# mbzuai-oryx/Video-LLaVA

Hardware: NVIDIA H100
Metric: videos/sec (100-frame CLIP encode + 7B 32-tok decode) (higher is better)
Workload: dtype bf16

## Files before the change

video-llava_b200/csrc/attention_tc.cu:

```cuda
#include "common.cuh"
#include "kernels.h"

#include <stdlib.h>

namespace vcl {

namespace {

constexpr int VA_WG = 2;
constexpr int VA_THREADS = VA_WG * 128;
constexpr int VA_TILE = 64 * 128;
constexpr int VA_KEY_TILES = 5;
constexpr int VA_OFF_K = 0;
constexpr int VA_OFF_VT = VA_OFF_K + VA_KEY_TILES * VA_TILE;
constexpr int VA_OFF_Q = VA_OFF_VT + VA_KEY_TILES * VA_TILE;
constexpr int VA_OFF_P = VA_OFF_Q + VA_WG * VA_TILE;
constexpr int VA_OFF_BAR = VA_OFF_P + VA_WG * VA_KEY_TILES * VA_TILE;
constexpr int VA_SMEM = VA_OFF_BAR + 64 + 1024;
static_assert(VA_SMEM <= 227 * 1024, "shared memory");

__device__ __forceinline__ uint32_t va_sw128(int row, int chunk) {
  return (uint32_t)row * 128u + (uint32_t)((chunk ^ (row & 7)) << 4);
}

__device__ __forceinline__ void named_bar_sync_wg(int id) { asm volatile("bar.sync %0, 128;" ::"r"(id) : "memory"); }

__global__ void __launch_bounds__(VA_THREADS, 1)
attn_vit_tc_kernel(const __grid_constant__ CUtensorMap tmap, const bf16* __restrict__ qkv, bf16* __restrict__ out,
                   int S, int H, int C) {
  extern __shared__ uint8_t smem_raw[];
  const uint32_t raw_addr = smem_u32(smem_raw);
  const uint32_t pad = ((raw_addr + 1023u) & ~1023u) - raw_addr;
  uint8_t* smem = smem_raw + pad;
  const uint32_t sbase = raw_addr + pad;
  const uint32_t kbar = sbase + VA_OFF_BAR;
  auto qbar = [&](int w) { return sbase + VA_OFF_BAR + 8u * (1 + w); };

  const int frame = blockIdx.x / H, h = blockIdx.x - frame * H;
  const int row0 = frame * S;
  const int wg = threadIdx.x >> 7, t = threadIdx.x & 127, lane = threadIdx.x & 31, wq = t >> 5;
  const int n_qt = (S + 63) / 64;
  const int n_kt = (S + 63) / 64;

  if (threadIdx.x == 0) {
    tma_prefetch_desc(&tmap);
    mbar_init(kbar, 1);
    for (int w = 0; w < VA_WG; ++w) mbar_init(qbar(w), 1);
    mbar_fence_init();
  }
  __syncthreads();
  if (threadIdx.x == 0) {
    mbar_arrive_expect_tx(kbar, n_kt * VA_TILE);
    for (int i = 0; i < n_kt; ++i) tma_load_2d(sbase + VA_OFF_K + i * VA_TILE, &tmap, kbar, C + h * 64, row0 + 64 * i);
    for (int w = 0; w < VA_WG && w < n_qt; ++w) {
      mbar_arrive_expect_tx(qbar(w), VA_TILE);
      tma_load_2d(sbase + VA_OFF_Q + w * VA_TILE, &tmap, qbar(w), h * 64, row0 + 64 * w);
    }
  }
  const bf16* vg = qkv + (long long)row0 * 3 * C + 2 * C + h * 64;
  for (int idx = threadIdx.x; idx < VA_KEY_TILES * 64 * 8; idx += VA_THREADS) {
    const int key = idx % (VA_KEY_TILES * 64), c = idx / (VA_KEY_TILES * 64);
    uint4 v = make_uint4(0u, 0u, 0u, 0u);
    if (key < S) v = *reinterpret_cast<const uint4*>(vg + (long long)key * 3 * C + c * 8);
    const uint32_t w4[4] = {v.x, v.y, v.z, v.w};
    uint8_t* tile = smem + VA_OFF_VT + (key >> 6) * VA_TILE;
    const int kc = (key & 63) >> 3, ke = key & 7;
#pragma unroll
    for (int e = 0; e < 8; ++e) {
      const uint16_t hv = (uint16_t)(e & 1 ? w4[e >> 1] >> 16 : w4[e >> 1] & 0xffffu);
      *reinterpret_cast<uint16_t*>(tile + va_sw128(c * 8 + e, kc) + ke * 2) = hv;
    }
  }
  asm volatile("fence.proxy.async.shared::cta;" ::: "memory");
  __syncthreads();
  mbar_wait(kbar, 0);

  const int r0 = 16 * wq + (lane >> 2), c2 = 2 * (lane & 3);
  const bool tail = S > 256;
  uint8_t* P = smem + VA_OFF_P + wg * VA_KEY_TILES * VA_TILE;
  const uint32_t p_addr = sbase + VA_OFF_P + wg * VA_KEY_TILES * VA_TILE;
  const uint32_t q_addr = sbase + VA_OFF_Q + wg * VA_TILE;
  uint32_t qphase = 0;
  float s[128], s2[16], o[32];
  for (int qt = wg; qt < n_qt; qt += VA_WG) {
    mbar_wait(qbar(wg), qphase);
    qphase ^= 1u;
#pragma unroll
    for (int i = 0; i < 128; ++i) s[i] = 0.f;
#pragma unroll
    for (int i = 0; i < 16; ++i) s2[i] = 0.f;
    wgmma_fence();
#pragma unroll
    for (int k = 0; k < 4; ++k) {
      const uint64_t ad = wgmma_desc_k_sw128(q_addr) + 2u * k;
      wgmma_bf16<256>(s, ad, wgmma_desc_k_sw128(sbase + VA_OFF_K) + 2u * k, k > 0 ? 1u : 0u);
      if (tail) wgmma_bf16<32>(s2, ad, wgmma_desc_k_sw128(sbase + VA_OFF_K + 256 * 128) + 2u * k, k > 0 ? 1u : 0u);
    }
    wgmma_commit();
    wgmma_wait<0>();
    wgmma_fence_regs(s);
    wgmma_fence_regs(s2);
    named_bar_sync_wg(1 + wg);
    if (t == 0 && qt + VA_WG < n_qt) {
      mbar_arrive_expect_tx(qbar(wg), VA_TILE);
      tma_load_2d(q_addr, &tmap, qbar(wg), h * 64, row0 + 64 * (qt + VA_WG));
    }
    auto sc = [&](float x, int key) { return key < S ? bf16r(bf16r(x) * 0.125f) : -INFINITY; };
    float m[2] = {-INFINITY, -INFINITY};
    uint32_t sp[64], sp2[8];
    auto pack_sc = [&](const float* a, int i, int key0) {
      const int hh = i & 1, col = key0 + 8 * (i >> 1) + c2;
      const float x0 = sc(a[2 * i], col), x1 = sc(a[2 * i + 1], col + 1);
      m[hh] = fmaxf(m[hh], fmaxf(x0, x1));
      return pack_bf16x2(x0, x1);
    };
    if (tail) {
#pragma unroll
      for (int i = 0; i < 8; ++i) sp2[i] = pack_sc(s2, i, 256);
    }
#pragma unroll
    for (int i = 0; i < 64; ++i) sp[i] = pack_sc(s, i, 0);
    float l[2] = {0.f, 0.f};
#pragma unroll
    for (int r = 0; r < 2; ++r) {
      m[r] = fmaxf(m[r], __shfl_xor_sync(0xffffffffu, m[r], 1));
      m[r] = fmaxf(m[r], __shfl_xor_sync(0xffffffffu, m[r], 2));
    }
    auto put_p = [&](uint32_t x2, int i, int key0) {
      const int hh = i & 1, row = r0 + 8 * hh, col = key0 + 8 * (i >> 1) + c2;
      const float p0 = exp2f((bf16lo(x2) - m[hh]) * 1.4426950408889634f);
      const float p1 = exp2f((bf16hi(x2) - m[hh]) * 1.4426950408889634f);
      l[hh] += p0 + p1;
      *reinterpret_cast<uint32_t*>(P + (col >> 6) * VA_TILE + va_sw128(row, (col & 63) >> 3) + (col & 7) * 2) =
          pack_bf16x2(p0, p1);
    };
#pragma unroll
    for (int i = 0; i < 64; ++i) put_p(sp[i], i, 0);
    if (tail) {
#pragma unroll
      for (int i = 0; i < 8; ++i) put_p(sp2[i], i, 256);
    }
    asm volatile("fence.proxy.async.shared::cta;" ::: "memory");
    named_bar_sync_wg(1 + wg);
#pragma unroll
    for (int i = 0; i < 32; ++i) o[i] = 0.f;
    wgmma_fence();
#pragma unroll
    for (int kk = 0; kk < 16; ++kk)
      wgmma_bf16<64>(o, wgmma_desc_k_sw128(p_addr + (kk >> 2) * VA_TILE) + 2u * (kk & 3),
                     wgmma_desc_k_sw128(sbase + VA_OFF_VT + (kk >> 2) * VA_TILE) + 2u * (kk & 3), kk > 0 ? 1u : 0u);
    if (tail)
      wgmma_bf16<64>(o, wgmma_desc_k_sw128(p_addr + 4 * VA_TILE), wgmma_desc_k_sw128(sbase + VA_OFF_VT + 4 * VA_TILE), 1u);
    wgmma_commit();
    wgmma_wait<0>();
    wgmma_fence_regs(o);
#pragma unroll
    for (int r = 0; r < 2; ++r) {
      l[r] += __shfl_xor_sync(0xffffffffu, l[r], 1);
      l[r] += __shfl_xor_sync(0xffffffffu, l[r], 2);
    }
#pragma unroll
    for (int hh = 0; hh < 2; ++hh) {
      const int q = qt * 64 + r0 + 8 * hh;
      if (q < S) {
        const float inv = 1.0f / l[hh];
        bf16* dst = out + (long long)(row0 + q) * C + h * 64 + c2;
#pragma unroll
        for (int j = 0; j < 8; ++j)
          *reinterpret_cast<uint32_t*>(dst + 8 * j) = pack_bf16x2(o[4 * j + 2 * hh] * inv, o[4 * j + 2 * hh + 1] * inv);
      }
    }
  }
}

}

int init_attention_tc_kernels() {
  VCL_CUDA_OK(cudaFuncSetAttribute(attn_vit_tc_kernel, cudaFuncAttributeMaxDynamicSharedMemorySize, VA_SMEM));
  return 0;
}

bool attention_vit_tc_supported(int S) {
  const bool off = getenv("VCL_VIT_ATTN_FLASH") != nullptr;
  return !off && S >= 129 && S <= 257;
}

int launch_attention_vit_tc(const bf16* qkv, bf16* out, int n_frames, int S, int H, int C, cudaStream_t stream) {
  VCL_REQUIRE(C == H * 64, "attention_vit_tc: head_dim must be 64");
  VCL_REQUIRE(S >= 129 && S <= 257, "attention_vit_tc: S=%d outside 129..257", S);
  VCL_REQUIRE(((uintptr_t)qkv % 16) == 0 && ((uintptr_t)out % 16) == 0, "attention_vit_tc: pointers must be 16-byte aligned");
  CUtensorMap tm;
  if (make_tmap_2d(&tm, qkv, (long long)n_frames * S, 3LL * C, 3LL * C, 64) != 0) return -2;
  attn_vit_tc_kernel<<<n_frames * H, VA_THREADS, VA_SMEM, stream>>>(tm, qkv, out, S, H, C);
  VCL_CUDA_OK(cudaGetLastError());
  count_launches(1);
  return 0;
}

}
```

video-llava_b200/csrc/common.cuh:

```cuda
#pragma once

#include <cuda.h>
#include <cuda_bf16.h>
#include <cuda_fp16.h>
#include <cuda_runtime.h>
#include <stdint.h>

namespace vcl {

typedef __nv_bfloat16 bf16;

void set_last_error(const char* fmt, ...);

#define VCL_CUDA_OK(expr)                                                                      \
  do {                                                                                         \
    cudaError_t _e = (expr);                                                                   \
    if (_e != cudaSuccess) {                                                                   \
      ::vcl::set_last_error("%s:%d: %s -> %s", __FILE__, __LINE__, #expr, cudaGetErrorString(_e)); \
      return -2;                                                                               \
    }                                                                                          \
  } while (0)

#define VCL_REQUIRE(cond, ...)                 \
  do {                                         \
// ... 26 lines not shown
  for (int o = 16; o > 0; o >>= 1) v += __shfl_xor_sync(0xffffffffu, v, o);
  return v;
}
__device__ __forceinline__ float warp_max(float v) {
#pragma unroll
  for (int o = 16; o > 0; o >>= 1) v = fmaxf(v, __shfl_xor_sync(0xffffffffu, v, o));
  return v;
}

__device__ __forceinline__ uint4 ld_nc_v4(const void* p) {
  uint4 r;
  asm volatile("ld.global.nc.L1::no_allocate.v4.u32 {%0,%1,%2,%3}, [%4];"
               : "=r"(r.x), "=r"(r.y), "=r"(r.z), "=r"(r.w)
               : "l"(p));
  return r;
}

__device__ __forceinline__ uint32_t smem_u32(const void* p) {
  return static_cast<uint32_t>(__cvta_generic_to_shared(p));
}

__device__ __forceinline__ void mbar_init(uint32_t bar, uint32_t count) {
  asm volatile("mbarrier.init.shared::cta.b64 [%0], %1;" ::"r"(bar), "r"(count) : "memory");
}
__device__ __forceinline__ void mbar_fence_init() {
  asm volatile("fence.mbarrier_init.release.cluster;" ::: "memory");
  asm volatile("fence.proxy.async.shared::cta;" ::: "memory");
}
__device__ __forceinline__ void mbar_arrive_expect_tx(uint32_t bar, uint32_t bytes) {
  asm volatile("mbarrier.arrive.expect_tx.shared::cta.b64 _, [%0], %1;" ::"r"(bar), "r"(bytes)
               : "memory");
}
__device__ __forceinline__ void mbar_arrive(uint32_t bar) {
  asm volatile("mbarrier.arrive.shared::cta.b64 _, [%0];" ::"r"(bar) : "memory");
}
__device__ __forceinline__ void mbar_wait(uint32_t bar, uint32_t parity) {
  asm volatile(
      "{\n\t"
      ".reg .pred p;\n\t"
      "VCL_WAIT_%=:\n\t"
      "mbarrier.try_wait.parity.shared::cta.b64 p, [%0], %1;\n\t"
      "@p bra VCL_DONE_%=;\n\t"
      "bra VCL_WAIT_%=;\n\t"
      "VCL_DONE_%=:\n\t"
      "}\n" ::"r"(bar),
      "r"(parity)
      : "memory");
}

__device__ __forceinline__ void tma_prefetch_desc(const void* tmap) {
  asm volatile("prefetch.tensormap [%0];" ::"l"(tmap) : "memory");
}
__device__ __forceinline__ void tma_load_2d(uint32_t dst_smem, const void* tmap, uint32_t bar,
                                            int32_t c0, int32_t c1) {
  asm volatile(
      "cp.async.bulk.tensor.2d.shared::cluster.global.mbarrier::complete_tx::bytes"
      " [%0], [%1, {%3, %4}], [%2];" ::"r"(dst_smem),
      "l"(tmap), "r"(bar), "r"(c0), "r"(c1)
      : "memory");
}

__device__ __forceinline__ void tma_prefetch_2d(const void* tmap, int32_t c0, int32_t c1) {
  asm volatile("cp.async.bulk.prefetch.tensor.2d.L2.global.tile [%0, {%1, %2}];" ::"l"(tmap), "r"(c0), "r"(c1)
               : "memory");
}

__device__ __forceinline__ void tma_load_2d_mc(uint32_t dst_smem, const void* tmap, uint32_t bar,
                                               int32_t c0, int32_t c1, uint16_t cta_mask) {
  asm volatile(
      "cp.async.bulk.tensor.2d.shared::cluster.global.mbarrier::complete_tx::bytes.multicast::cluster"
      " [%0], [%1, {%3, %4}], [%2], %5;" ::"r"(dst_smem),
      "l"(tmap), "r"(bar), "r"(c0), "r"(c1), "h"(cta_mask)
      : "memory");
}

__device__ __forceinline__ uint32_t cluster_ctarank() {
  uint32_t r;
  asm volatile("mov.u32 %0, %%cluster_ctarank;" : "=r"(r));
  return r;
}
__device__ __forceinline__ void cluster_sync_all() {
  asm volatile("barrier.cluster.arrive.release.aligned;" ::: "memory");
  asm volatile("barrier.cluster.wait.acquire.aligned;" ::: "memory");
}

__device__ __forceinline__ uint32_t mapa_cluster(uint32_t smem_addr, uint32_t cta_rank) {
  uint32_t r;
  asm volatile("mapa.shared::cluster.u32 %0, %1, %2;" : "=r"(r) : "r"(smem_addr), "r"(cta_rank));
  return r;
}
__device__ __forceinline__ void mbar_arrive_cluster(uint32_t bar_cluster_addr) {
  asm volatile("mbarrier.arrive.release.cluster.shared::cluster.b64 _, [%0];" ::"r"(bar_cluster_addr) : "memory");
}

__device__ __forceinline__ void wgmma_fence() { asm volatile("wgmma.fence.sync.aligned;" ::: "memory"); }
__device__ __forceinline__ void wgmma_commit() { asm volatile("wgmma.commit_group.sync.aligned;" ::: "memory"); }
template <int N>
__device__ __forceinline__ void wgmma_wait() {
  asm volatile("wgmma.wait_group.sync.aligned %0;" ::"n"(N) : "memory");
}
template <int R>
__device__ __forceinline__ void wgmma_fence_regs(float (&d)[R]) {
#pragma unroll
  for (int i = 0; i < R; ++i) asm volatile("" : "+f"(d[i])::"memory");
}
template <int R>
__device__ __forceinline__ void setmaxnreg_inc() { asm volatile("setmaxnreg.inc.sync.aligned.u32 %0;" ::"n"(R)); }
template <int R>
__device__ __forceinline__ void setmaxnreg_dec() { asm volatile("setmaxnreg.dec.sync.aligned.u32 %0;" ::"n"(R)); }

__device__ __forceinline__ uint64_t wgmma_desc_k_sw128(uint32_t smem_addr) {
  uint64_t d = 0;
  d |= (uint64_t)((smem_addr & 0x3ffffu) >> 4);
  d |= (uint64_t)1 << 16;
  d |= (uint64_t)(1024u >> 4) << 32;
  d |= (uint64_t)1 << 62;
  return d;
}

template <int N>
__device__ __forceinline__ void wgmma_bf16(float (&d)[N / 2], uint64_t adesc, uint64_t bdesc, uint32_t accumulate);
template <>
__device__ __forceinline__ void wgmma_bf16<256>(float (&d)[128], uint64_t adesc, uint64_t bdesc, uint32_t accumulate) {
  asm volatile(
      "{\n\t.reg .pred p;\n\tsetp.ne.b32 p, %130, 0;\n\t"
      "wgmma.mma_async.sync.aligned.m64n256k16.f32.bf16.bf16 {%0, %1, %2, %3, %4, %5, %6, %7, %8, %9, %10, %11, %12, %13, %14, %15, %16, %17, %18, %19, %20, %21, %22, %23, %24, %25, %26, %27, %28, %29, %30, %31, %32, %33, %34, %35, %36, %37, %38, %39, %40, %41, %42, %43, %44, %45, %46, %47, %48, %49, %50, %51, %52, %53, %54, %55, %56, %57, %58, %59, %60, %61, %62, %63, %64, %65, %66, %67, %68, %69, %70, %71, %72, %73, %74, %75, %76, %77, %78, %79, %80, %81, %82, %83, %84, %85, %86, %87, %88, %89, %90, %91, %92, %93, %94, %95, %96, %97, %98, %99, %100, %101, %102, %103, %104, %105, %106, %107, %108, %109, %110, %111, %112, %113, %114, %115, %116, %117, %118, %119, %120, %121, %122, %123, %124, %125, %126, %127}, %128, %129, p, 1, 1, 0, 0;\n\t}"
      : "+f"(d[0]), "+f"(d[1]), "+f"(d[2]), "+f"(d[3]), "+f"(d[4]), "+f"(d[5]), "+f"(d[6]), "+f"(d[7]), "+f"(d[8]), "+f"(d[9]), "+f"(d[10]), "+f"(d[11]), "+f"(d[12]), "+f"(d[13]), "+f"(d[14]), "+f"(d[15]), "+f"(d[16]), "+f"(d[17]), "+f"(d[18]), "+f"(d[19]), "+f"(d[20]), "+f"(d[21]), "+f"(d[22]), "+f"(d[23]), "+f"(d[24]), "+f"(d[25]), "+f"(d[26]), "+f"(d[27]), "+f"(d[28]), "+f"(d[29]), "+f"(d[30]), "+f"(d[31]), "+f"(d[32]), "+f"(d[33]), "+f"(d[34]), "+f"(d[35]), "+f"(d[36]), "+f"(d[37]), "+f"(d[38]), "+f"(d[39]), "+f"(d[40]), "+f"(d[41]), "+f"(d[42]), "+f"(d[43]), "+f"(d[44]), "+f"(d[45]), "+f"(d[46]), "+f"(d[47]), "+f"(d[48]), "+f"(d[49]), "+f"(d[50]), "+f"(d[51]), "+f"(d[52]), "+f"(d[53]), "+f"(d[54]), "+f"(d[55]), "+f"(d[56]), "+f"(d[57]), "+f"(d[58]), "+f"(d[59]), "+f"(d[60]), "+f"(d[61]), "+f"(d[62]), "+f"(d[63]), "+f"(d[64]), "+f"(d[65]), "+f"(d[66]), "+f"(d[67]), "+f"(d[68]), "+f"(d[69]), "+f"(d[70]), "+f"(d[71]), "+f"(d[72]), "+f"(d[73]), "+f"(d[74]), "+f"(d[75]), "+f"(d[76]), "+f"(d[77]), "+f"(d[78]), "+f"(d[79]), "+f"(d[80]), "+f"(d[81]), "+f"(d[82]), "+f"(d[83]), "+f"(d[84]), "+f"(d[85]), "+f"(d[86]), "+f"(d[87]), "+f"(d[88]), "+f"(d[89]), "+f"(d[90]), "+f"(d[91]), "+f"(d[92]), "+f"(d[93]), "+f"(d[94]), "+f"(d[95]), "+f"(d[96]), "+f"(d[97]), "+f"(d[98]), "+f"(d[99]), "+f"(d[100]), "+f"(d[101]), "+f"(d[102]), "+f"(d[103]), "+f"(d[104]), "+f"(d[105]), "+f"(d[106]), "+f"(d[107]), "+f"(d[108]), "+f"(d[109]), "+f"(d[110]), "+f"(d[111]), "+f"(d[112]), "+f"(d[113]), "+f"(d[114]), "+f"(d[115]), "+f"(d[116]), "+f"(d[117]), "+f"(d[118]), "+f"(d[119]), "+f"(d[120]), "+f"(d[121]), "+f"(d[122]), "+f"(d[123]), "+f"(d[124]), "+f"(d[125]), "+f"(d[126]), "+f"(d[127])
      : "l"(adesc), "l"(bdesc), "r"(accumulate));
}
template <>
__device__ __forceinline__ void wgmma_bf16<128>(float (&d)[64], uint64_t adesc, uint64_t bdesc, uint32_t accumulate) {
  asm volatile(
      "{\n\t.reg .pred p;\n\tsetp.ne.b32 p, %66, 0;\n\t"
      "wgmma.mma_async.sync.aligned.m64n128k16.f32.bf16.bf16 {%0, %1, %2, %3, %4, %5, %6, %7, %8, %9, %10, %11, %12, %13, %14, %15, %16, %17, %18, %19, %20, %21, %22, %23, %24, %25, %26, %27, %28, %29, %30, %31, %32, %33, %34, %35, %36, %37, %38, %39, %40, %41, %42, %43, %44, %45, %46, %47, %48, %49, %50, %51, %52, %53, %54, %55, %56, %57, %58, %59, %60, %61, %62, %63}, %64, %65, p, 1, 1, 0, 0;\n\t}"
      : "+f"(d[0]), "+f"(d[1]), "+f"(d[2]), "+f"(d[3]), "+f"(d[4]), "+f"(d[5]), "+f"(d[6]), "+f"(d[7]), "+f"(d[8]), "+f"(d[9]), "+f"(d[10]), "+f"(d[11]), "+f"(d[12]), "+f"(d[13]), "+f"(d[14]), "+f"(d[15]), "+f"(d[16]), "+f"(d[17]), "+f"(d[18]), "+f"(d[19]), "+f"(d[20]), "+f"(d[21]), "+f"(d[22]), "+f"(d[23]), "+f"(d[24]), "+f"(d[25]), "+f"(d[26]), "+f"(d[27]), "+f"(d[28]), "+f"(d[29]), "+f"(d[30]), "+f"(d[31]), "+f"(d[32]), "+f"(d[33]), "+f"(d[34]), "+f"(d[35]), "+f"(d[36]), "+f"(d[37]), "+f"(d[38]), "+f"(d[39]), "+f"(d[40]), "+f"(d[41]), "+f"(d[42]), "+f"(d[43]), "+f"(d[44]), "+f"(d[45]), "+f"(d[46]), "+f"(d[47]), "+f"(d[48]), "+f"(d[49]), "+f"(d[50]), "+f"(d[51]), "+f"(d[52]), "+f"(d[53]), "+f"(d[54]), "+f"(d[55]), "+f"(d[56]), "+f"(d[57]), "+f"(d[58]), "+f"(d[59]), "+f"(d[60]), "+f"(d[61]), "+f"(d[62]), "+f"(d[63])
      : "l"(adesc), "l"(bdesc), "r"(accumulate));
}
template <>
__device__ __forceinline__ void wgmma_bf16<64>(float (&d)[32], uint64_t adesc, uint64_t bdesc, uint32_t accumulate) {
  asm volatile(
      "{\n\t.reg .pred p;\n\tsetp.ne.b32 p, %34, 0;\n\t"
      "wgmma.mma_async.sync.aligned.m64n64k16.f32.bf16.bf16 {%0, %1, %2, %3, %4, %5, %6, %7, %8, %9, %10, %11, %12, %13, %14, %15, %16, %17, %18, %19, %20, %21, %22, %23, %24, %25, %26, %27, %28, %29, %30, %31}, %32, %33, p, 1, 1, 0, 0;\n\t}"
      : "+f"(d[0]), "+f"(d[1]), "+f"(d[2]), "+f"(d[3]), "+f"(d[4]), "+f"(d[5]), "+f"(d[6]), "+f"(d[7]), "+f"(d[8]), "+f"(d[9]), "+f"(d[10]), "+f"(d[11]), "+f"(d[12]), "+f"(d[13]), "+f"(d[14]), "+f"(d[15]), "+f"(d[16]), "+f"(d[17]), "+f"(d[18]), "+f"(d[19]), "+f"(d[20]), "+f"(d[21]), "+f"(d[22]), "+f"(d[23]), "+f"(d[24]), "+f"(d[25]), "+f"(d[26]), "+f"(d[27]), "+f"(d[28]), "+f"(d[29]), "+f"(d[30]), "+f"(d[31])
      : "l"(adesc), "l"(bdesc), "r"(accumulate));
}
template <>
__device__ __forceinline__ void wgmma_bf16<32>(float (&d)[16], uint64_t adesc, uint64_t bdesc, uint32_t accumulate) {
  asm volatile(
      "{\n\t.reg .pred p;\n\tsetp.ne.b32 p, %18, 0;\n\t"
      "wgmma.mma_async.sync.aligned.m64n32k16.f32.bf16.bf16 {%0, %1, %2, %3, %4, %5, %6, %7, %8, %9, %10, %11, %12, %13, %14, %15}, %16, %17, p, 1, 1, 0, 0;\n\t}"
      : "+f"(d[0]), "+f"(d[1]), "+f"(d[2]), "+f"(d[3]), "+f"(d[4]), "+f"(d[5]), "+f"(d[6]), "+f"(d[7]), "+f"(d[8]), "+f"(d[9]), "+f"(d[10]), "+f"(d[11]), "+f"(d[12]), "+f"(d[13]), "+f"(d[14]), "+f"(d[15])
      : "l"(adesc), "l"(bdesc), "r"(accumulate));
}

}
```

video-llava_b200/csrc/vcl_api.cu:

```cuda
#include "../../include/vcl.h"

#include <stdarg.h>
#include <stdio.h>
#include <stdlib.h>
#include <string.h>

#include <map>
#include <string>
#include <vector>

#include "common.cuh"
#include "kernels.h"

namespace vcl {

static thread_local char g_err[1024] = "";
static long long g_launches = 0;

void count_launches(long long n) { g_launches += n; }
long long launch_count() { return g_launches; }

void set_last_error(const char* fmt, ...) {
  va_list ap;
  va_start(ap, fmt);
// ... 199 lines not shown
  VCL_CUDA_OK(cudaMemset(bad, 0x7f, (size_t)n_mats * 2 * sizeof(int)));
  auto quant = [&](bf16* W, DecodeW& d, int N, int K, bool qkv, int idx) -> int {
    if (dalloc(h, &d.q, gemv_tiled_elems(N, K)) || dalloc(h, &d.s, (size_t)N)) return -2;
    return launch_gemv_quantize_fp8(W, W, d.q, d.s, N, K, qkv, bad + 2 * idx, nullptr);
  };
  int rc = 0;
  for (int l = 0; l < L && rc == 0; ++l) {
    LlmLayerW& w = h->ll[l];
    rc = quant(w.wqkv, w.qkv_d, 3 * D, D, true, 4 * l);
    if (rc == 0) rc = quant(w.wo, w.o_d, D, D, false, 4 * l + 1);
    if (rc == 0) rc = quant(w.wgu, w.gu_d, 2 * F, D, false, 4 * l + 2);
    if (rc == 0) rc = quant(w.wd, w.dn_d, D, F, false, 4 * l + 3);
  }
  if (rc == 0) rc = quant(h->lm_head, h->lm_head_d, c.vocab, D, false, 4 * L);
  std::vector<int> flags((size_t)n_mats * 2);
  cudaError_t e = cudaDeviceSynchronize();
  if (e == cudaSuccess) e = cudaMemcpy(flags.data(), bad, flags.size() * sizeof(int), cudaMemcpyDeviceToHost);
  cudaFree(bad);
  if (rc != 0) return rc;
  if (e != cudaSuccess) {
    set_last_error("vcl_load_llm_weights: %s", cudaGetErrorString(e));
    return -2;
  }
  auto name_of = [&](int idx, int r, int* row) -> std::string {
    if (idx == 4 * L) { *row = r; return "lm_head.weight"; }
    const std::string lp = "model.layers." + std::to_string(idx / 4) + ".";
    switch (idx % 4) {
      case 0: { static const char* nm[3] = {"q_proj", "k_proj", "v_proj"};
                *row = r % D; return lp + "self_attn." + nm[r / D] + ".weight"; }
      case 1: *row = r; return lp + "self_attn.o_proj.weight";
      case 2: *row = r / 2; return lp + (r % 2 ? "mlp.up_proj.weight" : "mlp.gate_proj.weight");
      default: *row = r; return lp + "mlp.down_proj.weight";
    }
  };
  for (int idx = 0; idx < n_mats; ++idx) {
    int row = 0;
    if (flags[2 * idx] != 0x7f7f7f7f) {
      const std::string nm = name_of(idx, flags[2 * idx], &row);
      VCL_REQUIRE(false, "weight '%s' has a non-finite value in row %d: the fp8 weight format needs finite weights",
                  nm.c_str(), row);
    }
    if (flags[2 * idx + 1] != 0x7f7f7f7f) {
      const std::string nm = name_of(idx, flags[2 * idx + 1], &row);
      VCL_REQUIRE(false, "weight '%s' row %d: its fp8 row scale 2^e is not a normal fp32 number or its dequantized "
                  "values are not exact bf16 numbers (a row maximum below ~1e-36)", nm.c_str(), row);
    }
  }
  return 0;
}

}

extern "C" {

int vcl_version(void) { return VCL_VERSION; }

const char* vcl_last_error(void) { return vcl::g_err; }

int vcl_create(vcl_handle** out, const vcl_config* c) {
  VCL_REQUIRE(out != nullptr && c != nullptr, "vcl_create: null argument");
  *out = nullptr;
  if (check_device() != 0) return -2;
  VCL_REQUIRE(c->clip_hidden > 0 && c->clip_heads > 0 && c->clip_hidden == c->clip_heads * 64,
              "vcl_create: CLIP head_dim must be 64 (hidden %d, heads %d)", c->clip_hidden, c->clip_heads);
  VCL_REQUIRE(c->clip_hidden % 256 == 0 && c->clip_inter % 256 == 0,
              "vcl_create: CLIP widths must be multiples of 256");
  VCL_REQUIRE(c->patch_size > 0 && c->image_size % c->patch_size == 0, "vcl_create: image/patch mismatch");
  VCL_REQUIRE(c->llm_hidden == c->llm_heads * 128, "vcl_create: LLM head_dim must be 128 (hidden %d, heads %d)",
              c->llm_hidden, c->llm_heads);
  VCL_REQUIRE(c->llm_hidden % 256 == 0 && c->llm_inter % 64 == 0, "vcl_create: LLM widths unsupported");
  VCL_REQUIRE(c->clip_layers >= 0 && c->llm_layers >= 0 && c->vocab > 0, "vcl_create: bad layer/vocab counts");
  VCL_REQUIRE(c->max_frames > 0 && c->max_batch > 0 && c->max_seq > 0, "vcl_create: capacities must be > 0");
  VCL_REQUIRE(c->proj_type == VCL_PROJ_LINEAR || c->proj_type == VCL_PROJ_MLP2X_GELU, "vcl_create: proj_type");
  VCL_REQUIRE(c->max_slots == 0 || (c->max_slots >= 1 && c->max_slots <= c->max_batch && c->max_slots <= 64),
              "vcl_create: max_slots=%d outside 1..%d (0: min(max_batch, 16))", c->max_slots,
              c->max_batch < 64 ? c->max_batch : 64);
  VCL_REQUIRE(c->kv_blocks == 0 || c->kv_blocks >= 2,
              "vcl_create: kv_blocks=%d: 0 (contiguous cache) or at least 2 (block 0 is the park block)", c->kv_blocks);
  {
    const int D = c->llm_hidden, F = c->llm_inter;
    const struct { const char* name; int N, K; bool norm; } mats[5] = {
        {"q|k|v", 3 * D, D, true}, {"o_proj", D, D, false}, {"gate|up", 2 * F, D, true},
        {"down_proj", D, F, false}, {"lm_head", c->vocab, D, true}};
    for (int B = 1; B <= c->max_batch && B <= 64; ++B)
      for (const auto& m : mats)
        VCL_REQUIRE(gemv_fits(B, m.N, m.K, m.norm),
                    "vcl_create: the %s projection [%d x %d] has no decode kernel for %d clips (1..4 clips: K <= 14336 "
                    "and the shared-memory plan)", m.name, m.N, m.K, B);
  }

  vcl_handle* h = new vcl_handle();
  h->cfg = *c;
  const int G = c->image_size / c->patch_size;
  h->P = G * G;
  h->KP = ((3 * c->patch_size * c->patch_size + 63) / 64) * 64;
  h->NV = c->n_temporal + h->P;

  int rc = 0;
  rc |= init_gemm_kernels();
  rc |= init_attention_kernels();
  rc |= init_gemv_kernels();

  const size_t C = c->clip_hidden, F = c->clip_inter;
  const size_t Mv = (size_t)c->max_frames * (h->P + 1);
  const size_t act_elems = Mv * F > (size_t)c->max_frames * h->P * h->KP ? Mv * F
                                                                          : (size_t)c->max_frames * h->P * h->KP;
  rc |= dalloc(h, &h->v_h, Mv * C);
  rc |= dalloc(h, &h->v_x, Mv * C);
  rc |= dalloc(h, &h->v_qkv, Mv * 3 * C);
  rc |= dalloc(h, &h->v_attn, Mv * C);
  rc |= dalloc(h, &h->v_act, act_elems);

  const size_t D = c->llm_hidden, LF = c->llm_inter;
  const size_t Ml = (size_t)c->max_batch * h->act_seq();
  rc |= dalloc(h, &h->l_h, Ml * D);
  rc |= dalloc(h, &h->l_x, Ml * D);
  rc |= dalloc(h, &h->l_qkv, Ml * 3 * D);
  rc |= dalloc(h, &h->l_attn, Ml * D);
  rc |= dalloc(h, &h->l_act, Ml * LF);
  rc |= dalloc(h, &h->l_vid, (size_t)c->max_batch * h->NV * D);
  rc |= dalloc(h, &h->l_vid_tmp, (size_t)c->max_batch * h->NV * D);
  if (h->paged()) {
    rc |= dalloc(h, &h->pool, (size_t)c->kv_blocks * h->block_elems());
    h->table_host.assign((size_t)h->n_slots_max() * h->table_row(), 0);
    rc |= dalloc(h, &h->d_table, h->table_host.size());
  } else {
    rc |= dalloc(h, &h->kcache, (size_t)c->llm_layers * h->cache_layer_elems());
    rc |= dalloc(h, &h->vcache, (size_t)c->llm_layers * h->cache_layer_elems());
  }
  rc |= dalloc(h, &h->rope_cos, (size_t)c->max_seq * 64);
  rc |= dalloc(h, &h->rope_sin, (size_t)c->max_seq * 64);
  rc |= dalloc(h, &h->logits, (size_t)c->max_batch * c->vocab);
  rc |= dalloc(h, &h->tokens, (size_t)c->max_batch * c->max_seq);
  const size_t Bm = c->max_batch;
  rc |= dalloc(h, &h->d_h, Bm * D);
  rc |= dalloc(h, &h->d_x, xwin_elems((int)Bm, (int)D) > Bm * D ? xwin_elems((int)Bm, (int)D) : Bm * D);
  rc |= dalloc(h, &h->d_q, Bm * D);
  rc |= dalloc(h, &h->d_qkv, Bm * 3 * D);
  rc |= dalloc(h, &h->d_attn, xwin_elems((int)Bm, (int)D) > Bm * D ? xwin_elems((int)Bm, (int)D) : Bm * D);
  rc |= dalloc(h, &h->d_act, xwin_elems((int)Bm, (int)LF) > Bm * LF ? xwin_elems((int)Bm, (int)LF) : Bm * LF);
  rc |= dalloc(h, &h->d_pos, Bm);
  rc |= dalloc(h, &h->d_npad, Bm);
  rc |= dalloc(h, &h->amax, (size_t)device_num_sms() * Bm);
  rc |= dalloc(h, &h->d_pack, pack_elems((long long)Ml));
  rc |= dalloc(h, &h->samp, Bm * 20);
  h->samp_host.assign(Bm * 20, 0);
  for (size_t b = 0; b < Bm; ++b) h->samp_topn(h->samp_host.data())[b] = -1;
  if (rc == 0) rc = launch_rope_table(h->rope_cos, h->rope_sin, c->max_seq, 128, c->rope_theta, 0);
  if (rc == 0) {
    cudaError_t e = cudaMemset(h->d_npad, 0, Bm * sizeof(int));
    if (e == cudaSuccess)
      e = cudaMemcpy(h->samp, h->samp_host.data(), h->samp_host.size(), cudaMemcpyHostToDevice);
    if (e == cudaSuccess && h->paged()) e = cudaMemset(h->d_table, 0, h->table_host.size() * sizeof(int));
    if (e == cudaSuccess) e = cudaDeviceSynchronize();
    if (e != cudaSuccess) {
      set_last_error("vcl_create: %s", cudaGetErrorString(e));
      rc = -2;
    }
  }
  if (rc != 0) {
    vcl_destroy(h);
    return -2;
  }
  *out = h;
  return 0;
}

void vcl_destroy(vcl_handle* h) {
  if (!h) return;
  for (auto& g : h->graphs) cudaGraphExecDestroy(g.exec);
  for (void* p : h->allocs) cudaFree(p);
  delete h;
}

int vcl_load_clip_weights(vcl_handle* h, const vcl_tensor* tensors, int n) {
  VCL_REQUIRE(h && tensors && n > 0, "vcl_load_clip_weights: null argument");
  VCL_REQUIRE(!h->clip_loaded, "vcl_load_clip_weights: already loaded");
  TensorMap m;
  for (int i = 0; i < n; ++i)
    if (tensors[i].name) m[tensors[i].name] = &tensors[i];
  const vcl_config& c = h->cfg;
  const long long C = c.clip_hidden, F = c.clip_inter, ps = c.patch_size;
  const std::string pre = "vision_model.";
  {
    const vcl_tensor* t = find_tensor(m, pre + "embeddings.patch_embedding.weight", 4, C, 3, ps, ps);
    if (!t) return -1;
    if (dalloc(h, &h->patch_w, (size_t)C * h->KP) != 0) return -2;
    VCL_CUDA_OK(cudaMemset(h->patch_w, 0, (size_t)C * h->KP * 2));
    const size_t k = 3 * ps * ps;
    VCL_CUDA_OK(cudaMemcpy2D(h->patch_w, (size_t)h->KP * 2, t->data, k * 2, k * 2, C,
                             cudaMemcpyDeviceToDevice));
  }
  if (load_copy(h, m, pre + "embeddings.class_embedding", &h->cls, 1, C)) return -1;
  if (load_copy(h, m, pre + "embeddings.position_embedding.weight", &h->pos, 2, h->P + 1, C)) return -1;
  if (load_copy(h, m, pre + "pre_layrnorm.weight", &h->pre_w, 1, C)) return -1;
  if (load_copy(h, m, pre + "pre_layrnorm.bias", &h->pre_b, 1, C)) return -1;
  h->cl.resize(c.clip_layers);
  for (int l = 0; l < c.clip_layers; ++l) {
    ClipLayerW& w = h->cl[l];
    const std::string lp = pre + "encoder.layers." + std::to_string(l) + ".";
    if (load_copy(h, m, lp + "layer_norm1.weight", &w.ln1_w, 1, C)) return -1;
    if (load_copy(h, m, lp + "layer_norm1.bias", &w.ln1_b, 1, C)) return -1;
    if (load_copy(h, m, lp + "layer_norm2.weight", &w.ln2_w, 1, C)) return -1;
    if (load_copy(h, m, lp + "layer_norm2.bias", &w.ln2_b, 1, C)) return -1;
    if (dalloc(h, &w.wqkv, (size_t)3 * C * C) || dalloc(h, &w.bqkv, (size_t)3 * C)) return -2;
    const char* nm[3] = {"q_proj", "k_proj", "v_proj"};
    for (int j = 0; j < 3; ++j) {
      const vcl_tensor* tw = find_tensor(m, lp + "self_attn." + nm[j] + ".weight", 2, C, C);
      const vcl_tensor* tb = find_tensor(m, lp + "self_attn." + nm[j] + ".bias", 1, C);
      if (!tw || !tb) return -1;
      VCL_CUDA_OK(cudaMemcpy(w.wqkv + (size_t)j * C * C, tw->data, (size_t)C * C * 2, cudaMemcpyDeviceToDevice));
      VCL_CUDA_OK(cudaMemcpy(w.bqkv + (size_t)j * C, tb->data, (size_t)C * 2, cudaMemcpyDeviceToDevice));
    }
    if (load_copy(h, m, lp + "self_attn.out_proj.weight", &w.wo, 2, C, C)) return -1;
    if (load_copy(h, m, lp + "self_attn.out_proj.bias", &w.bo, 1, C)) return -1;
    if (load_copy(h, m, lp + "mlp.fc1.weight", &w.w1, 2, F, C)) return -1;
    if (load_copy(h, m, lp + "mlp.fc1.bias", &w.b1, 1, F)) return -1;
    if (load_copy(h, m, lp + "mlp.fc2.weight", &w.w2, 2, C, F)) return -1;
    if (load_copy(h, m, lp + "mlp.fc2.bias", &w.b2, 1, C)) return -1;
  }
  VCL_CUDA_OK(cudaDeviceSynchronize());
  h->clip_loaded = true;
  return 0;
}

int vcl_load_llm_weights(vcl_handle* h, const vcl_tensor* tensors, int n) {
  return vcl_load_llm_weights_ex(h, tensors, n, VCL_WEIGHTS_BF16);
}

int vcl_load_llm_weights_ex(vcl_handle* h, const vcl_tensor* tensors, int n, int weight_format) {
  VCL_REQUIRE(weight_format == VCL_WEIGHTS_BF16 || weight_format == VCL_WEIGHTS_FP8_E4M3,
              "vcl_load_llm_weights: unknown weight format %d (VCL_WEIGHTS_BF16 0, VCL_WEIGHTS_FP8_E4M3 1)",
              weight_format);
  VCL_REQUIRE(h && tensors && n > 0, "vcl_load_llm_weights: null argument");
  VCL_REQUIRE(!h->llm_loaded, "vcl_load_llm_weights: already loaded");
  const bool fp8 = weight_format == VCL_WEIGHTS_FP8_E4M3;
  if (fp8) {
    const vcl_config& c = h->cfg;
    const int D = c.llm_hidden, F = c.llm_inter;
    const struct { const char* name; int N, K; bool norm; } mats[5] = {
        {"q|k|v", 3 * D, D, true}, {"o_proj", D, D, false}, {"gate|up", 2 * F, D, true},
        {"down_proj", D, F, false}, {"lm_head", c.vocab, D, true}};
    for (int B = 1; B <= c.max_batch && B <= 64; ++B)
      for (const auto& mt : mats)
        VCL_REQUIRE(gemv_fits(B, mt.N, mt.K, mt.norm, true),
                    "vcl_load_llm_weights: the %s projection [%d x %d] has no fp8 decode kernel for %d clips", mt.name,
                    mt.N, mt.K, B);
  }
  TensorMap m;
  for (int i = 0; i < n; ++i)
    if (tensors[i].name) m[tensors[i].name] = &tensors[i];
  const vcl_config& c = h->cfg;
  const long long D = c.llm_hidden, F = c.llm_inter, V = c.vocab, CV = c.clip_hidden;
  if (load_copy(h, m, "model.embed_tokens.weight", &h->embed, 2, V, D)) return -1;
  if (load_copy(h, m, "model.norm.weight", &h->norm_w, 1, D)) return -1;
  {
    const vcl_tensor* t = find_tensor(m, "lm_head.weight", 2, V, D);
    if (!t) return -1;
    const size_t Vp = h->vocab_padded();
    if (dalloc(h, &h->lm_head, Vp * D) != 0) return -2;
    VCL_CUDA_OK(cudaMemset(h->lm_head + (size_t)V * D, 0, (Vp - V) * D * sizeof(bf16)));
    VCL_CUDA_OK(cudaMemcpy(h->lm_head, t->data, (size_t)V * D * sizeof(bf16), cudaMemcpyDeviceToDevice));
  }
  if (c.proj_type == VCL_PROJ_LINEAR) {
    if (load_copy(h, m, "model.mm_projector.weight", &h->proj_w0, 2, D, CV)) return -1;
    if (load_copy(h, m, "model.mm_projector.bias", &h->proj_b0, 1, D)) return -1;
  } else {
    if (load_copy(h, m, "model.mm_projector.0.weight", &h->proj_w0, 2, D, CV)) return -1;
    if (load_copy(h, m, "model.mm_projector.0.bias", &h->proj_b0, 1, D)) return -1;
    if (load_copy(h, m, "model.mm_projector.2.weight", &h->proj_w1, 2, D, D)) return -1;
    if (load_copy(h, m, "model.mm_projector.2.bias", &h->proj_b1, 1, D)) return -1;
  }
  h->ll.resize(c.llm_layers);
  for (int l = 0; l < c.llm_layers; ++l) {
    LlmLayerW& w = h->ll[l];
    const std::string lp = "model.layers." + std::to_string(l) + ".";
    if (load_copy(h, m, lp + "input_layernorm.weight", &w.ln1, 1, D)) return -1;
    if (load_copy(h, m, lp + "post_attention_layernorm.weight", &w.ln2, 1, D)) return -1;
    if (dalloc(h, &w.wqkv, (size_t)3 * D * D)) return -2;
    const char* nm[3] = {"q_proj", "k_proj", "v_proj"};
    for (int j = 0; j < 3; ++j) {
      const vcl_tensor* tw = find_tensor(m, lp + "self_attn." + nm[j] + ".weight", 2, D, D);
      if (!tw) return -1;
      VCL_CUDA_OK(cudaMemcpy(w.wqkv + (size_t)j * D * D, tw->data, (size_t)D * D * 2, cudaMemcpyDeviceToDevice));
    }
    if (load_copy(h, m, lp + "self_attn.o_proj.weight", &w.wo, 2, D, D)) return -1;
    const vcl_tensor* tg = find_tensor(m, lp + "mlp.gate_proj.weight", 2, F, D);
    const vcl_tensor* tu = find_tensor(m, lp + "mlp.up_proj.weight", 2, F, D);
    if (!tg || !tu) return -1;
    if (dalloc(h, &w.wgu, (size_t)2 * F * D)) return -2;
    VCL_CUDA_OK(cudaMemcpy2D(w.wgu, (size_t)2 * D * 2, tg->data, (size_t)D * 2, (size_t)D * 2, F,
                             cudaMemcpyDeviceToDevice));
    VCL_CUDA_OK(cudaMemcpy2D(w.wgu + D, (size_t)2 * D * 2, tu->data, (size_t)D * 2, (size_t)D * 2, F,
                             cudaMemcpyDeviceToDevice));
    if (load_copy(h, m, lp + "mlp.down_proj.weight", &w.wd, 2, D, F)) return -1;
  }
  if (fp8) {
    VCL_TRY(quantize_llm_fp8(h));
    h->llm_loaded = true;
    return 0;
  }
  auto tiled = [&](const bf16* src, DecodeW& dst, int N, int K, bool qkv) -> int {
    if (dalloc(h, &dst.t, gemv_tiled_elems(N, K))) return -2;
    return launch_gemv_repack(src, dst.t, N, K, qkv, nullptr);
  };
  for (int l = 0; l < c.llm_layers; ++l) {
// ... 1082 lines not shown
```

Before: 5.062.

## Restructure ViT attention: register-sourced P, TMA V load, two CTAs per SM

```diff
diff --git a/video-llava_b200/csrc/attention_tc.cu b/video-llava_b200/csrc/attention_tc.cu
--- a/video-llava_b200/csrc/attention_tc.cu
+++ b/video-llava_b200/csrc/attention_tc.cu
@@ -1,156 +1,143 @@
 #include "common.cuh"
 #include "kernels.h"
-
-#include <stdlib.h>
 
 namespace vcl {
 
 namespace {
 
-constexpr int VA_WG = 2;
-constexpr int VA_THREADS = VA_WG * 128;
+constexpr int VA_THREADS = 128;
 constexpr int VA_TILE = 64 * 128;
 constexpr int VA_KEY_TILES = 5;
 constexpr int VA_OFF_K = 0;
-constexpr int VA_OFF_VT = VA_OFF_K + VA_KEY_TILES * VA_TILE;
-constexpr int VA_OFF_Q = VA_OFF_VT + VA_KEY_TILES * VA_TILE;
-constexpr int VA_OFF_P = VA_OFF_Q + VA_WG * VA_TILE;
-constexpr int VA_OFF_BAR = VA_OFF_P + VA_WG * VA_KEY_TILES * VA_TILE;
-constexpr int VA_SMEM = VA_OFF_BAR + 64 + 1024;
-static_assert(VA_SMEM <= 227 * 1024, "shared memory");
+constexpr int VA_OFF_V = VA_OFF_K + VA_KEY_TILES * VA_TILE;
+constexpr int VA_OFF_Q = VA_OFF_V + VA_KEY_TILES * VA_TILE;
+constexpr int VA_OFF_BAR = VA_OFF_Q + 2 * VA_TILE;
+constexpr int VA_SMEM = VA_OFF_BAR + 32 + 1024;
+static_assert(2 * (VA_SMEM + 1024) <= 228 * 1024, "two CTAs per SM");
 
-__device__ __forceinline__ uint32_t va_sw128(int row, int chunk) {
-  return (uint32_t)row * 128u + (uint32_t)((chunk ^ (row & 7)) << 4);
-}
-
-__device__ __forceinline__ void named_bar_sync_wg(int id) { asm volatile("bar.sync %0, 128;" ::"r"(id) : "memory"); }
-
-__global__ void __launch_bounds__(VA_THREADS, 1)
-attn_vit_tc_kernel(const __grid_constant__ CUtensorMap tmap, const bf16* __restrict__ qkv, bf16* __restrict__ out,
-                   int S, int H, int C) {
+template <bool TAIL>
+__global__ void __launch_bounds__(VA_THREADS, 2)
+attn_vit_tc_kernel(const __grid_constant__ CUtensorMap tmap, bf16* __restrict__ out, int S, int H, int C) {
   extern __shared__ uint8_t smem_raw[];
   const uint32_t raw_addr = smem_u32(smem_raw);
   const uint32_t pad = ((raw_addr + 1023u) & ~1023u) - raw_addr;
   uint8_t* smem = smem_raw + pad;
   const uint32_t sbase = raw_addr + pad;
-  const uint32_t kbar = sbase + VA_OFF_BAR;
-  auto qbar = [&](int w) { return sbase + VA_OFF_BAR + 8u * (1 + w); };
+  const uint32_t kbar = sbase + VA_OFF_BAR, vbar = kbar + 8;
+  auto qbar = [&](int slot) { return kbar + 16u + 8u * slot; };
 
   const int frame = blockIdx.x / H, h = blockIdx.x - frame * H;
   const int row0 = frame * S;
-  const int wg = threadIdx.x >> 7, t = threadIdx.x & 127, lane = threadIdx.x & 31, wq = t >> 5;
+  const int t = threadIdx.x, lane = t & 31, wq = t >> 5;
   const int n_qt = (S + 63) / 64;
-  const int n_kt = (S + 63) / 64;
+  constexpr int KV_END = TAIL ? 272 : 256;
 
-  if (threadIdx.x == 0) {
+  if (t == 0) {
     tma_prefetch_desc(&tmap);
     mbar_init(kbar, 1);
-    for (int w = 0; w < VA_WG; ++w) mbar_init(qbar(w), 1);
+    mbar_init(vbar, 1);
+    mbar_init(qbar(0), 1);
+    mbar_init(qbar(1), 1);
     mbar_fence_init();
+    mbar_arrive_expect_tx(qbar(0), VA_TILE);
+    tma_load_2d(sbase + VA_OFF_Q, &tmap, qbar(0), h * 64, row0);
+    mbar_arrive_expect_tx(kbar, n_qt * VA_TILE);
+    for (int i = 0; i < n_qt; ++i) tma_load_2d(sbase + VA_OFF_K + i * VA_TILE, &tmap, kbar, C + h * 64, row0 + 64 * i);
+    mbar_arrive_expect_tx(vbar, n_qt * VA_TILE);
+    for (int i = 0; i < n_qt; ++i) tma_load_2d(sbase + VA_OFF_V + i * VA_TILE, &tmap, vbar, 2 * C + h * 64, row0 + 64 * i);
+    mbar_arrive_expect_tx(qbar(1), VA_TILE);
+    tma_load_2d(sbase + VA_OFF_Q + VA_TILE, &tmap, qbar(1), h * 64, row0 + 64);
   }
   __syncthreads();
-  if (threadIdx.x == 0) {
-    mbar_arrive_expect_tx(kbar, n_kt * VA_TILE);
-    for (int i = 0; i < n_kt; ++i) tma_load_2d(sbase + VA_OFF_K + i * VA_TILE, &tmap, kbar, C + h * 64, row0 + 64 * i);
-    for (int w = 0; w < VA_WG && w < n_qt; ++w) {
-      mbar_arrive_expect_tx(qbar(w), VA_TILE);
-      tma_load_2d(sbase + VA_OFF_Q + w * VA_TILE, &tmap, qbar(w), h * 64, row0 + 64 * w);
-    }
-  }
-  const bf16* vg = qkv + (long long)row0 * 3 * C + 2 * C + h * 64;
-  for (int idx = threadIdx.x; idx < VA_KEY_TILES * 64 * 8; idx += VA_THREADS) {
-    const int key = idx % (VA_KEY_TILES * 64), c = idx / (VA_KEY_TILES * 64);
-    uint4 v = make_uint4(0u, 0u, 0u, 0u);
-    if (key < S) v = *reinterpret_cast<const uint4*>(vg + (long long)key * 3 * C + c * 8);
-    const uint32_t w4[4] = {v.x, v.y, v.z, v.w};
-    uint8_t* tile = smem + VA_OFF_VT + (key >> 6) * VA_TILE;
-    const int kc = (key & 63) >> 3, ke = key & 7;
-#pragma unroll
-    for (int e = 0; e < 8; ++e) {
-      const uint16_t hv = (uint16_t)(e & 1 ? w4[e >> 1] >> 16 : w4[e >> 1] & 0xffffu);
-      *reinterpret_cast<uint16_t*>(tile + va_sw128(c * 8 + e, kc) + ke * 2) = hv;
-    }
-  }
-  asm volatile("fence.proxy.async.shared::cta;" ::: "memory");
-  __syncthreads();
-  mbar_wait(kbar, 0);
 
   const int r0 = 16 * wq + (lane >> 2), c2 = 2 * (lane & 3);
-  const bool tail = S > 256;
-  uint8_t* P = smem + VA_OFF_P + wg * VA_KEY_TILES * VA_TILE;
-  const uint32_t p_addr = sbase + VA_OFF_P + wg * VA_KEY_TILES * VA_TILE;
-  const uint32_t q_addr = sbase + VA_OFF_Q + wg * VA_TILE;
-  uint32_t qphase = 0;
-  float s[128], s2[16], o[32];
-  for (int qt = wg; qt < n_qt; qt += VA_WG) {
-    mbar_wait(qbar(wg), qphase);
-    qphase ^= 1u;
+  for (int qt = 0; qt < n_qt; ++qt) {
+    const int slot = qt & 1;
+    const uint32_t q_addr = sbase + VA_OFF_Q + slot * VA_TILE;
+    mbar_wait(qbar(slot), (qt >> 1) & 1);
+    if (qt == 0) mbar_wait(kbar, 0);
+    float s[128], s2[4];
 #pragma unroll
     for (int i = 0; i < 128; ++i) s[i] = 0.f;
 #pragma unroll
-    for (int i = 0; i < 16; ++i) s2[i] = 0.f;
+    for (int i = 0; i < 4; ++i) s2[i] = 0.f;
     wgmma_fence();
 #pragma unroll
     for (int k = 0; k < 4; ++k) {
       const uint64_t ad = wgmma_desc_k_sw128(q_addr) + 2u * k;
       wgmma_bf16<256>(s, ad, wgmma_desc_k_sw128(sbase + VA_OFF_K) + 2u * k, k > 0 ? 1u : 0u);
-      if (tail) wgmma_bf16<32>(s2, ad, wgmma_desc_k_sw128(sbase + VA_OFF_K + 256 * 128) + 2u * k, k > 0 ? 1u : 0u);
+      if constexpr (TAIL)
+        wgmma_bf16<8>(s2, ad, wgmma_desc_k_sw128(sbase + VA_OFF_K + 256 * 128) + 2u * k, k > 0 ? 1u : 0u);
     }
     wgmma_commit();
     wgmma_wait<0>();
     wgmma_fence_regs(s);
     wgmma_fence_regs(s2);
-    named_bar_sync_wg(1 + wg);
-    if (t == 0 && qt + VA_WG < n_qt) {
-      mbar_arrive_expect_tx(qbar(wg), VA_TILE);
-      tma_load_2d(q_addr, &tmap, qbar(wg), h * 64, row0 + 64 * (qt + VA_WG));
+    __syncthreads();
+    if (t == 0 && qt + 2 < n_qt) {
+      mbar_arrive_expect_tx(qbar(slot), VA_TILE);
+      tma_load_2d(q_addr, &tmap, qbar(slot), h * 64, row0 + 64 * (qt + 2));
     }
-    auto sc = [&](float x, int key) { return key < S ? bf16r(bf16r(x) * 0.125f) : -INFINITY; };
-    float m[2] = {-INFINITY, -INFINITY};
-    uint32_t sp[64], sp2[8];
-    auto pack_sc = [&](const float* a, int i, int key0) {
-      const int hh = i & 1, col = key0 + 8 * (i >> 1) + c2;
-      const float x0 = sc(a[2 * i], col), x1 = sc(a[2 * i + 1], col + 1);
-      m[hh] = fmaxf(m[hh], fmaxf(x0, x1));
-      return pack_bf16x2(x0, x1);
-    };
-    if (tail) {
+    uint32_t p[64], p2[2] = {0u, 0u};
+    float l[2] = {0.f, 0.f};
+    if (qt * 64 + 16 * wq < S) {
+      const int s_keys = TAIL ? 257 : S;
+      auto sc = [&](float x, int key) { return key < s_keys ? bf16r(bf16r(x) * 0.125f) : -INFINITY; };
+      float m[2] = {-INFINITY, -INFINITY};
+      auto scale_pair = [&](float* a, int i, int key0) {
+        const int hh = i & 1, col = key0 + 8 * (i >> 1) + c2;
+        a[2 * i] = sc(a[2 * i], col);
+        a[2 * i + 1] = sc(a[2 * i + 1], col + 1);
+        m[hh] = fmaxf(m[hh], fmaxf(a[2 * i], a[2 * i + 1]));
+      };
+      if constexpr (TAIL) {
 #pragma unroll
-      for (int i = 0; i < 8; ++i) sp2[i] = pack_sc(s2, i, 256);
+        for (int i = 0; i < 2; ++i) scale_pair(s2, i, 256);
+      }
+#pragma unroll
+      for (int i = 0; i < 64; ++i) scale_pair(s, i, 0);
+#pragma unroll
+      for (int r = 0; r < 2; ++r) {
+        m[r] = fmaxf(m[r], __shfl_xor_sync(0xffffffffu, m[r], 1));
+        m[r] = fmaxf(m[r], __shfl_xor_sync(0xffffffffu, m[r], 2));
+      }
+      auto exp_p = [&](const float* a, int i) {
+        const int hh = i & 1;
+        const float p0 = exp2f((a[2 * i] - m[hh]) * 1.4426950408889634f);
+        const float p1 = exp2f((a[2 * i + 1] - m[hh]) * 1.4426950408889634f);
+        l[hh] += p0 + p1;
+        return pack_bf16x2(p0, p1);
+      };
+#pragma unroll
+      for (int i = 0; i < 64; ++i) p[i] = exp_p(s, i);
+      if constexpr (TAIL) {
+#pragma unroll
+        for (int i = 0; i < 2; ++i) p2[i] = exp_p(s2, i);
+      }
+    } else {
+#pragma unroll
+      for (int i = 0; i < 64; ++i) p[i] = 0u;
     }
-#pragma unroll
-    for (int i = 0; i < 64; ++i) sp[i] = pack_sc(s, i, 0);
-    float l[2] = {0.f, 0.f};
-#pragma unroll
-    for (int r = 0; r < 2; ++r) {
-      m[r] = fmaxf(m[r], __shfl_xor_sync(0xffffffffu, m[r], 1));
-      m[r] = fmaxf(m[r], __shfl_xor_sync(0xffffffffu, m[r], 2));
+    if (qt == 0) {
+      mbar_wait(vbar, 0);
+      for (int off = S * 128 + 16 * t; off < KV_END * 128; off += 16 * VA_THREADS)
+        *reinterpret_cast<uint4*>(smem + VA_OFF_V + off) = make_uint4(0u, 0u, 0u, 0u);
+      asm volatile("fence.proxy.async.shared::cta;" ::: "memory");
+      __syncthreads();
     }
-    auto put_p = [&](uint32_t x2, int i, int key0) {
-      const int hh = i & 1, row = r0 + 8 * hh, col = key0 + 8 * (i >> 1) + c2;
-      const float p0 = exp2f((bf16lo(x2) - m[hh]) * 1.4426950408889634f);
-      const float p1 = exp2f((bf16hi(x2) - m[hh]) * 1.4426950408889634f);
-      l[hh] += p0 + p1;
-      *reinterpret_cast<uint32_t*>(P + (col >> 6) * VA_TILE + va_sw128(row, (col & 63) >> 3) + (col & 7) * 2) =
-          pack_bf16x2(p0, p1);
-    };
-#pragma unroll
-    for (int i = 0; i < 64; ++i) put_p(sp[i], i, 0);
-    if (tail) {
-#pragma unroll
-      for (int i = 0; i < 8; ++i) put_p(sp2[i], i, 256);
-    }
-    asm volatile("fence.proxy.async.shared::cta;" ::: "memory");
-    named_bar_sync_wg(1 + wg);
+    float o[32];
 #pragma unroll
     for (int i = 0; i < 32; ++i) o[i] = 0.f;
     wgmma_fence();
 #pragma unroll
-    for (int kk = 0; kk < 16; ++kk)
-      wgmma_bf16<64>(o, wgmma_desc_k_sw128(p_addr + (kk >> 2) * VA_TILE) + 2u * (kk & 3),
-                     wgmma_desc_k_sw128(sbase + VA_OFF_VT + (kk >> 2) * VA_TILE) + 2u * (kk & 3), kk > 0 ? 1u : 0u);
-    if (tail)
-      wgmma_bf16<64>(o, wgmma_desc_k_sw128(p_addr + 4 * VA_TILE), wgmma_desc_k_sw128(sbase + VA_OFF_VT + 4 * VA_TILE), 1u);
+    for (int kk = 0; kk < 16; ++kk) {
+      const uint32_t a[4] = {p[4 * kk], p[4 * kk + 1], p[4 * kk + 2], p[4 * kk + 3]};
+      wgmma_bf16_rs_n64_mn(o, a, wgmma_desc_k_sw128(sbase + VA_OFF_V + kk * 16 * 128), kk > 0 ? 1u : 0u);
+    }
+    if constexpr (TAIL) {
+      const uint32_t a[4] = {p2[0], p2[1], 0u, 0u};
+      wgmma_bf16_rs_n64_mn(o, a, wgmma_desc_k_sw128(sbase + VA_OFF_V + 256 * 128), 1u);
+    }
     wgmma_commit();
     wgmma_wait<0>();
     wgmma_fence_regs(o);
@@ -176,14 +163,12 @@
 }
 
 int init_attention_tc_kernels() {
-  VCL_CUDA_OK(cudaFuncSetAttribute(attn_vit_tc_kernel, cudaFuncAttributeMaxDynamicSharedMemorySize, VA_SMEM));
+  VCL_CUDA_OK(cudaFuncSetAttribute(attn_vit_tc_kernel<false>, cudaFuncAttributeMaxDynamicSharedMemorySize, VA_SMEM));
+  VCL_CUDA_OK(cudaFuncSetAttribute(attn_vit_tc_kernel<true>, cudaFuncAttributeMaxDynamicSharedMemorySize, VA_SMEM));
   return 0;
 }
 
-bool attention_vit_tc_supported(int S) {
-  const bool off = getenv("VCL_VIT_ATTN_FLASH") != nullptr;
-  return !off && S >= 129 && S <= 257;
-}
+bool attention_vit_tc_supported(int S) { return S >= 129 && S <= 257; }
 
 int launch_attention_vit_tc(const bf16* qkv, bf16* out, int n_frames, int S, int H, int C, cudaStream_t stream) {
   VCL_REQUIRE(C == H * 64, "attention_vit_tc: head_dim must be 64");
@@ -191,7 +176,10 @@
   VCL_REQUIRE(((uintptr_t)qkv % 16) == 0 && ((uintptr_t)out % 16) == 0, "attention_vit_tc: pointers must be 16-byte aligned");
   CUtensorMap tm;
   if (make_tmap_2d(&tm, qkv, (long long)n_frames * S, 3LL * C, 3LL * C, 64) != 0) return -2;
-  attn_vit_tc_kernel<<<n_frames * H, VA_THREADS, VA_SMEM, stream>>>(tm, qkv, out, S, H, C);
+  if (S > 256)
+    attn_vit_tc_kernel<true><<<n_frames * H, VA_THREADS, VA_SMEM, stream>>>(tm, out, S, H, C);
+  else
+    attn_vit_tc_kernel<false><<<n_frames * H, VA_THREADS, VA_SMEM, stream>>>(tm, out, S, H, C);
   VCL_CUDA_OK(cudaGetLastError());
   count_launches(1);
   return 0;
diff --git a/video-llava_b200/csrc/common.cuh b/video-llava_b200/csrc/common.cuh
--- a/video-llava_b200/csrc/common.cuh
+++ b/video-llava_b200/csrc/common.cuh
@@ -202,5 +202,22 @@
       : "+f"(d[0]), "+f"(d[1]), "+f"(d[2]), "+f"(d[3]), "+f"(d[4]), "+f"(d[5]), "+f"(d[6]), "+f"(d[7]), "+f"(d[8]), "+f"(d[9]), "+f"(d[10]), "+f"(d[11]), "+f"(d[12]), "+f"(d[13]), "+f"(d[14]), "+f"(d[15])
       : "l"(adesc), "l"(bdesc), "r"(accumulate));
 }
-
-}
+template <>
+__device__ __forceinline__ void wgmma_bf16<8>(float (&d)[4], uint64_t adesc, uint64_t bdesc, uint32_t accumulate) {
+  asm volatile(
+      "{\n\t.reg .pred p;\n\tsetp.ne.b32 p, %6, 0;\n\t"
+      "wgmma.mma_async.sync.aligned.m64n8k16.f32.bf16.bf16 {%0, %1, %2, %3}, %4, %5, p, 1, 1, 0, 0;\n\t}"
+      : "+f"(d[0]), "+f"(d[1]), "+f"(d[2]), "+f"(d[3])
+      : "l"(adesc), "l"(bdesc), "r"(accumulate));
+}
+
+__device__ __forceinline__ void wgmma_bf16_rs_n64_mn(float (&d)[32], const uint32_t (&a)[4], uint64_t bdesc,
+                                                     uint32_t accumulate) {
+  asm volatile(
+      "{\n\t.reg .pred p;\n\tsetp.ne.b32 p, %37, 0;\n\t"
+      "wgmma.mma_async.sync.aligned.m64n64k16.f32.bf16.bf16 {%0, %1, %2, %3, %4, %5, %6, %7, %8, %9, %10, %11, %12, %13, %14, %15, %16, %17, %18, %19, %20, %21, %22, %23, %24, %25, %26, %27, %28, %29, %30, %31}, {%32, %33, %34, %35}, %36, p, 1, 1, 1;\n\t}"
+      : "+f"(d[0]), "+f"(d[1]), "+f"(d[2]), "+f"(d[3]), "+f"(d[4]), "+f"(d[5]), "+f"(d[6]), "+f"(d[7]), "+f"(d[8]), "+f"(d[9]), "+f"(d[10]), "+f"(d[11]), "+f"(d[12]), "+f"(d[13]), "+f"(d[14]), "+f"(d[15]), "+f"(d[16]), "+f"(d[17]), "+f"(d[18]), "+f"(d[19]), "+f"(d[20]), "+f"(d[21]), "+f"(d[22]), "+f"(d[23]), "+f"(d[24]), "+f"(d[25]), "+f"(d[26]), "+f"(d[27]), "+f"(d[28]), "+f"(d[29]), "+f"(d[30]), "+f"(d[31])
+      : "r"(a[0]), "r"(a[1]), "r"(a[2]), "r"(a[3]), "l"(bdesc), "r"(accumulate));
+}
+
+}
diff --git a/video-llava_b200/csrc/vcl_api.cu b/video-llava_b200/csrc/vcl_api.cu
--- a/video-llava_b200/csrc/vcl_api.cu
+++ b/video-llava_b200/csrc/vcl_api.cu
@@ -375,6 +375,12 @@
     if (e == cudaSuccess)
       e = cudaMemcpy(h->samp, h->samp_host.data(), h->samp_host.size(), cudaMemcpyHostToDevice);
     if (e == cudaSuccess && h->paged()) e = cudaMemset(h->d_table, 0, h->table_host.size() * sizeof(int));
+    if (e == cudaSuccess && h->paged()) e = cudaMemset(h->pool, 0, (size_t)c->kv_blocks * h->block_elems() * sizeof(bf16));
+    if (e == cudaSuccess && !h->paged()) {
+      const size_t bytes = (size_t)c->llm_layers * h->cache_layer_elems() * sizeof(bf16);
+      e = cudaMemset(h->kcache, 0, bytes);
+      if (e == cudaSuccess) e = cudaMemset(h->vcache, 0, bytes);
+    }
     if (e == cudaSuccess) e = cudaDeviceSynchronize();
     if (e != cudaSuccess) {
       set_last_error("vcl_create: %s", cudaGetErrorString(e));
```

New measurement: 5.128, median of 6. +1.3%, better.
